# oksuman/FHE-Sorting

Hardware: AMD Instinct MI355X
Metric: encrypted sort seconds + ciphertext-mults/sec, N=1024 @ ringDim 2^16 (higher is better)
Workload: dtype u64; 1 GPU; DirectSort N=1024, ringDim 2^16, depth 39, scale 2^40, 161 rotation keys, CompositeSign(3, 5, 2), dnum 3, OpenFHE PS split; N=1024, ring_dim=65536, mult_depth=39, scale_bits=40, ps_split=openfhe, special_primes=10, lanes_per_gpu=2, max_stack=32, parallelism=batch-shard x1, collective=none

## Files before the change

### fhe-sorting_amd/csrc/capi/capi.cpp

```cpp
#include <hip/hip_runtime.h>
#include <rccl/rccl.h>
#include <sys/random.h>

#include <cerrno>
#include <cstdlib>
#include <cstring>
#include <map>
#include <memory>
#include <new>
#include <string>

#include "../../../include/fhe_gpu.h"
#include "../algo/bootstrap.hpp"
#include "../algo/fhesort.hpp"
#include "../device/kernels.hpp"
#include "../algo/kway.hpp"
#include "../engine/engine.hpp"
#include "../wire/wire.hpp"

using namespace fhe;

struct fhe_ctx {
    std::unique_ptr<Engine> eng;
    wire::CtxParams params;
// ... 158 lines not shown
    });
}
int fhe_key_is_seeded(fhe_ctx *ctx, uint64_t galois) {
    int r = -FHE_EINVAL;
    const int st = guard([&] {
        NEED(ctx);
        r = ctx->eng->key_seeded(galois);
        if (r < 0) {
            g_err = "fhe_key_is_seeded: no such key";
            r = -FHE_ENOKEY;
        }
    });
    return st == FHE_OK ? r : -st;
}
int fhe_public_poly(fhe_ctx *ctx, const uint8_t seed[32], uint64_t kid, int digit, uint64_t *out) {
    return guard([&] {
        NEED(ctx);
        NEED(seed);
        NEED(out);
        ctx->eng->public_poly(seed, kid, digit, out);
    });
}
uint64_t fhe_key_bytes(fhe_ctx *ctx) { return ctx ? ctx->eng->key_bytes() : 0; }

int fhe_encrypt(fhe_ctx *ctx, const double *v, int len, int slots, int level, fhe_ct **out) {
    return guard([&] { *out = wrap(ctx->eng->encrypt(std::vector<double>(v, v + len), slots, level)); });
}
int fhe_encrypt_ext(fhe_ctx *ctx, const double *v, int len, int slots, fhe_ct **out) {
    return guard([&] { *out = wrap(ctx->eng->encrypt_ext(std::vector<double>(v, v + len), slots)); });
}
int fhe_decrypt(fhe_ctx *ctx, const fhe_ct *ct, double *out) {
    return guard([&] {
        auto v = ctx->eng->decrypt(*ct->p);
        std::memcpy(out, v.data(), v.size() * 8);
    });
}
int fhe_ct_upload(fhe_ctx *ctx, const uint64_t *h, int limbs, int level, int slots, double scale, fhe_ct **out) {
    return guard([&] { *out = wrap(ctx->eng->upload(h, (size_t)limbs, level, slots, scale)); });
}
int fhe_ct_download(fhe_ctx *ctx, const fhe_ct *ct, uint64_t *h) {
    return guard([&] { ctx->eng->download(*ct->p, h); });
}
int fhe_ct_info(const fhe_ct *ct, int *level, int *slots, double *scale, int *limbs) {
    return guard([&] {
        NEED(ct);
        if (level) *level = ct->p->level;
// ... 1624 lines not shown
```

### fhe-sorting_amd/csrc/device/kernels.hpp

```cpp
#pragma once
#include <string>
#include <utility>
#include <vector>
#include <hip/hip_runtime.h>
#include <hip/hip_ext.h>
#include <cstddef>
#include <cstdint>

#include "modmath.hpp"

namespace fhe {
namespace dev {

struct NttTables {
    const ulonglong2 *fwd2;
    const ulonglong2 *inv2;
    const u64 *ninv, *ninv_s;
    const Mod *mods;
    int logN;
    const double *fwdd = nullptr, *invd = nullptr;
    const double2 *qd = nullptr;
    const uint8_t *fp_host = nullptr;
};
bool ntt_fp_prime(u64 q);
// ... 166 lines not shown

void encode_ifft(double2 *v, int64_t *coef, int B, int S, int n, const double2 *ksi, const uint32_t *rot,
                 const double *scale, unsigned *overflow, hipStream_t st);
void mask_slots(double2 *v, int B, int S, int N, const int *spec, hipStream_t st);
void select_slots(double2 *vc, double2 *vk, int S, int N, const int *targets, int count, int shift, hipStream_t st);
void tiebreak_slots(double2 *v, int B, int S, int N, const int *batches, double eps, hipStream_t st);

int set_mfma_sums(int mask);
void modup_convert(u64 *ext, const u64 *coef, int ell, int K, int alpha, int digits, int members,
                   size_t coef_stride, size_t ext_stride, const int *pmap_ext,
                   const u64 *tabs , const size_t *tab_off, const Mod *mods, int logN,
                   hipStream_t st,
                   const double *fptab = nullptr, const size_t *fp_off = nullptr, int fpmid = -1);
struct KsStrides {
    size_t acc = 0, ext = 0, d = 0;
    int zs0 = 0, zn0 = 1 << 30, zs1 = 0;
    __host__ __device__ int target_of(int z) const { return z < zn0 ? zs0 + z : zs1 + (z - zn0); }
};
struct KsFold {
    const u64 *d = nullptr;
    size_t seg = 0, member = 0;
    u64 w = 0, ws = 0;
};
void ks_inner(u64 *acc, const u64 *ext, const u64 *dntt, const u64 *key, int ell, int K, int nq, int nall,
              int alpha, int digits, const uint32_t *perm, const int *pmap_ext, const Mod *mods, int logN,
              hipStream_t st, int members, KsStrides str, KsFold fold = KsFold(), int tcount = -1);
void ntt_forward_mapped_cols(u64 *data, int count, int segs, size_t seg, const int *smap, const int *pmap,
                             const NttTables &T, hipStream_t st);
void ntt_row_ks(u64 *acc, const u64 *ext, const u64 *dntt, const u64 *key, int ell, int K, int nall, int alpha,
                int digits, const int *pmap_ext, int members, KsStrides str, KsFold fold, const NttTables &T,
                hipStream_t st, bool fp_only = false, int tfirst = 0);
void ntt_forward_mapped_rows(u64 *data, int count, int segs, size_t seg, const int *smap, const int *pmap,
                             const NttTables &T, hipStream_t st);
std::vector<std::pair<int, int>> ntt_class_runs(const int *pmap, int count, bool fp, const NttTables &T);
constexpr int KS_MAXKEYS = 16;
struct KsKeys {
    const u64 *key[KS_MAXKEYS];
    const uint32_t *perm[KS_MAXKEYS];
};
void ks_inner_multikey_sum(u64 *acc, const u64 *ext, const u64 *dntt, const KsKeys &keys, int count, bool accumulate,
                           int ell, int K, int nall, int alpha, int digits, const int *pmap_ext, const Mod *mods,
                           int logN, hipStream_t st, KsStrides str);
constexpr int LT_MAXB = 16;
struct LtArgs {
    const u64 *key[LT_MAXB];
    const uint32_t *perm[LT_MAXB];
    const u64 *pt[LT_MAXB];
    int nb;
};
void lt_inner(u64 *out, const u64 *ext, const u64 *c, const LtArgs &A, bool accumulate, int ell, int K, int nall,
              int alpha, int digits, const int *pmap_ext, const u64 *pmodq, const u64 *pmodq_s, const Mod *mods,
              int logN, hipStream_t st);
void ew_permute_sum(u64 *out, const u64 *in, const KsKeys &keys, int limbs, int count, bool accumulate, size_t in_stride,
                    const Mod *mods, int logN, hipStream_t st);
// ... 40 lines not shown
```

### fhe-sorting_amd/csrc/device/ntt.hip

```cpp
#include <hip/hip_ext.h>

#include <cstdlib>
#include <map>
#include <atomic>
#include <mutex>
#include <stdexcept>
#include <string>
#include <type_traits>
#include <utility>
#include <vector>

#include "kernels.hpp"

namespace fhe {
namespace dev {

namespace {

constexpr int NTB = 256;

template <int Lo, int Hi, typename F>
void dispatch_int(int v, F &&f) {
    if constexpr (Lo > Hi) {
        throw std::invalid_argument("unsupported digit count " + std::to_string(v));
// ... 879 lines not shown
#endif
#ifndef FHE_NTT_FP_ROW_WPE
#define FHE_NTT_FP_ROW_WPE 1
#endif
#ifndef FHE_NTT_FP_RESCALE_WPE
#define FHE_NTT_FP_RESCALE_WPE FHE_NTT_FP_ROW_WPE
#endif
template <int MODE, bool FULL, bool TWL, bool FP>
__global__ __launch_bounds__(NTB) __attribute__((amdgpu_waves_per_eu(FP ? (MODE == NTT_RESCALE ? FHE_NTT_FP_RESCALE_WPE : FHE_NTT_FP_ROW_WPE) : TWL ? FHE_NTT_ROW_WPE : 1, 8))) void k_ntt_fwd_row(
    u64 *data, size_t seg, const int *pmap, const int *smap, int logN, NttTables Tb, NttFuse F) {
    ntt_fwd_body<8, 4, false, MODE, true, FULL, TWL, FP>(data, seg, pmap, smap, logN, Tb, F, blockIdx.z);
}
template <bool FULL, bool TWL, bool FP>
__global__ __launch_bounds__(NTB) __attribute__((amdgpu_waves_per_eu(TWL ? FHE_NTT_ROW_WPE : 1, 8))) void k_ntt_inv_row(
    u64 *data, size_t seg, const int *pmap, const int *smap, int logN, NttTables Tb, NttFuse F) {
    ntt_inv_body<8, 4, false, true, FULL, TWL, FP>(data, seg, pmap, smap, logN, Tb, F);
}
#ifndef FHE_ROW_KS_WPE
#define FHE_ROW_KS_WPE 2
#endif
#ifndef FHE_ROW_KS_WPE1
#define FHE_ROW_KS_WPE1 4
#endif
template <int D, bool FP, bool FULL>
__global__ __launch_bounds__(NTB) __attribute__((amdgpu_waves_per_eu(D == 1 ? FHE_ROW_KS_WPE1 : FHE_ROW_KS_WPE, 8))) void k_ntt_row_ks(u64 *acc, const u64 *ext, const u64 *dntt, const u64 *key,
                                                    int ell, int W, int nall, int alpha, int members,
                                                    const int *pmap_ext, int logN, NttTables Tb, KsStrides st,
                                                    KsFold fold, NttFuse Fz, int lmb) {
    using TW = TwT<FP>;
    __shared__ TW twl[TWL_ROWS * 256];
    const size_t n = (size_t)1 << logN;
    const int t = Fz.limb_of(blockIdx.z);
    const int pt = __builtin_amdgcn_readfirstlane(pmap_ext[t]);
    const int tr = threadIdx.x >> 4, tl = threadIdx.x & 15;
    const int R = 16 >> lmb;
    const int mb = ((int)blockIdx.x << lmb) + (tr & ((1 << lmb) - 1));
    const bool valid = FULL || mb < members;
    const size_t row0 = (size_t)blockIdx.y * R, row = row0 + (tr >> lmb), rb = row * 256;
    const Mod md = Tb.mods[pt];
    const u64 q = md.q, q2 = 2 * q;
    Ar A{4 * q, (u64)0 - q, 0.0, 0.0};
    const TW *tw;
    if constexpr (FP) {
        tw = Tb.fwdd + (size_t)pt * n;
        const double2 qd = Tb.qd[pt];
        A.q = qd.x;
        A.qi = qd.y;
    } else {
        tw = Tb.fwd2 + (size_t)pt * n;
    }
    const int S0 = logN - 8;
    row_twiddles_multi<true>(twl, tw, row0, R, n, S0);
    __syncthreads();
    const TW *twr = twl + 256 * (tr >> lmb);
    const size_t m = valid ? (size_t)mb : 0;
    const int li = row_final_index<true>(tl, 0);
#define IDX(r) (li + (row_final_index<true>(0, r)))
    const bool folded = fold.d && t == ell - 1;
    const u64 *fd = fold.d + m * fold.member;
    auto digit_row = [&](int j, u64(&x)[16]) {
        const int lo = j * alpha, hi = min((j + 1) * alpha, ell);
        if (t >= lo && t < hi) {
            const u64 *src = dntt + m * st.d + (size_t)t * n + rb;
#pragma unroll
            for (int r = 0; r < 16; ++r) {
                const u64 v = valid ? src[IDX(r)] : 0;
                x[r] = FP ? ubits(fp_in(v, FP_TWO52)) : v;
            }
        } else {
            const u64 *src = ext + m * st.ext + ((size_t)j * W + t) * n + rb;
            const double fin = FP ? FP_TWO52 + FP_FWD_COL_OUT * A.q : 0.0;
#pragma unroll
            for (int r = 0; r < 16; ++r) {
                const u64 v = valid ? src[tl + 16 * r] : 0;
                x[r] = FP ? ubits(fp_in(v, fin)) : v;
            }
            row_pass_shfl<true, true, FP>(x, tl, row, twr, n, S0, A);
            if constexpr (!FP) {
#pragma unroll
                for (int r = 0; r < 16; ++r) x[r] = canon12(x[r], q, q2);
            }
        }
    };
    auto mac = [&](int j, const u64(&x)[16], u64(&a0)[16], u64(&a1)[16]) {
        const u64 *kb = key + (((size_t)j * 2 + 0) * nall + pt) * n + rb;
        const u64 *ka = key + (((size_t)j * 2 + 1) * nall + pt) * n + rb;
#pragma unroll
        for (int r = 0; r < 16; ++r) {
            const u64 b = kb[IDX(r)], c = ka[IDX(r)];
            if constexpr (FP) {
                const double xv = dbits(x[r]);
                a0[r] = ubits(dbits(a0[r]) + fp_mulmod(xv, fp_in(b, FP_TWO52), A.q, A.qi));
                a1[r] = ubits(dbits(a1[r]) + fp_mulmod(xv, fp_in(c, FP_TWO52), A.q, A.qi));
            } else {
                a0[r] = add_mod(a0[r], mul_barrett(x[r], b, md), q);
                a1[r] = add_mod(a1[r], mul_barrett(x[r], c, md), q);
            }
        }
    };
    auto fold_of = [&](int r, u64 &f0, u64 &f1) {
        f0 = f1 = 0;
        if (folded && valid) {
            f0 = mul_shoup(fd[rb + IDX(r)], fold.w, fold.ws, q);
            f1 = mul_shoup(fd[fold.seg + rb + IDX(r)], fold.w, fold.ws, q);
        }
    };
    u64 *o0 = acc + m * st.acc + (size_t)t * n + rb;
    u64 *o1 = acc + m * st.acc + ((size_t)W + t) * n + rb;
    auto fin = [&](u64 v) -> u64 {
        if constexpr (FP) {
            const double r0 = fp_reduce(dbits(v), A.q, A.qi);
            return fp_out(r0 < 0.0 ? r0 + A.q : r0, FP_TWO52);
        } else {
            return v;
        }
    };
    if constexpr (D == 1) {
        u64 x[16];
        digit_row(0, x);
        const u64 *kb = key + (size_t)pt * n + rb;
        const u64 *ka = key + ((size_t)nall + pt) * n + rb;
#pragma unroll
        for (int r = 0; r < 16; ++r) {
            u64 f0, f1, v0, v1;
            fold_of(r, f0, f1);
            const u64 b = kb[IDX(r)], c = ka[IDX(r)];
            if constexpr (FP) {
                const double xv = dbits(x[r]);
                v0 = ubits(fp_in(f0, FP_TWO52) + fp_mulmod(xv, fp_in(b, FP_TWO52), A.q, A.qi));
                v1 = ubits(fp_in(f1, FP_TWO52) + fp_mulmod(xv, fp_in(c, FP_TWO52), A.q, A.qi));
            } else {
                v0 = add_mod(f0, mul_barrett(x[r], b, md), q);
                v1 = add_mod(f1, mul_barrett(x[r], c, md), q);
            }
            if (valid) {
                o0[IDX(r)] = fin(v0);
                o1[IDX(r)] = fin(v1);
            }
        }
        return;
    }
    u64 a0[16], a1[16];
#pragma unroll
    for (int r = 0; r < 16; ++r) {
        u64 f0, f1;
        fold_of(r, f0, f1);
        a0[r] = FP ? ubits(fp_in(f0, FP_TWO52)) : f0;
        a1[r] = FP ? ubits(fp_in(f1, FP_TWO52)) : f1;
    }
#pragma unroll 1
    for (int j = 0; j < D; ++j) {
        u64 x[16];
        digit_row(j, x);
        mac(j, x, a0, a1);
    }
    if (!valid) return;
#pragma unroll
    for (int r = 0; r < 16; ++r) {
        o0[IDX(r)] = fin(a0[r]);
        o1[IDX(r)] = fin(a1[r]);
    }
#undef IDX
}

int &row_twl_enabled() {
    static int v = [] {
        const char *e = std::getenv("FHE_NTT_TWL");
        return e ? std::atoi(e) : 1;
    }();
    return v;
}

int &row_twl_rows() {
    static int v = [] {
        const char *e = std::getenv("FHE_NTT_TWL_ROWS");
        return e ? std::atoi(e) : 4;
    }();
    return v;
}
// ... 401 lines not shown
void ntt_forward_mapped_rows(u64 *data, int count, int segs, size_t seg, const int *smap, const int *pmap,
                             const NttTables &T, hipStream_t st) {
    if (count <= 0 || segs <= 0) return;
    const int k2 = T.logN - (T.logN + 1) / 2;
    const NttFuse F;
    dispatch<false, true, NTT_PLAIN>(k2, data, count, segs, seg, pmap, smap, T, F, st);
}

std::vector<std::pair<int, int>> ntt_class_runs(const int *pmap, int count, bool fp, const NttTables &T) {
    std::vector<int> pr;
    const bool known = launch_primes(pmap, count, pr);
    std::vector<std::pair<int, int>> runs;
    for (int z = 0; z < count; ++z) {
        const bool f = ntt_fp_enabled() && T.fp_host && known && T.fp_host[pr[z]] != 0;
        if (f != fp) continue;
        if (!runs.empty() && runs.back().first + runs.back().second == z) ++runs.back().second;
        else runs.emplace_back(z, 1);
    }
    return runs;
}

void ntt_row_ks(u64 *acc, const u64 *ext, const u64 *dntt, const u64 *key, int ell, int K, int nall, int alpha,
                int digits, const int *pmap_ext, int members, KsStrides str, KsFold fold, const NttTables &T,
                hipStream_t st, bool fp_only, int tfirst) {
    const int W = ell + K;
    if (T.logN != 16 && T.logN != 17) throw std::invalid_argument("ntt_row_ks: the row pass is 256 points (rings 2^16, 2^17)");
    if (digits < 1 || digits > 8) throw std::invalid_argument("ntt_row_ks: 1..8 digits");
    if (members < 1) return;
    std::vector<int> pr;
    const bool known = launch_primes(pmap_ext, W, pr);
    (void)pr;
    if (!known && ntt_fp_enabled() && T.fp_host) throw std::invalid_argument("ntt_row_ks: unregistered prime map");
    int lmb = 4;
    while (lmb > 2 && (1 << lmb) > members) --lmb;
    const bool full = members % (1 << lmb) == 0;
    const dim3 blk(NTB);
    for (int cls = fp_only ? 1 : 0; cls < 2; ++cls) {
        std::vector<std::pair<int, int>> runs;
        for (auto r : ntt_class_runs(pmap_ext, W, cls == 1, T)) {
            const int lo = std::max(r.first, tfirst), hi = r.first + r.second;
            if (lo < hi) runs.emplace_back(lo, hi - lo);
        }
        for (size_t r = 0; r < runs.size(); r += 2) {
            NttFuse Fz;
            Fz.zs0 = runs[r].first;
            Fz.zn0 = runs[r].second;
            Fz.zs1 = r + 1 < runs.size() ? runs[r + 1].first : 0;
            const int cnt = runs[r].second + (r + 1 < runs.size() ? runs[r + 1].second : 0);
            const dim3 grid((unsigned)((members + (1 << lmb) - 1) >> lmb), (unsigned)((1u << (T.logN - 8)) >> (4 - lmb)),
                            (unsigned)cnt);
            const double bytes = 8.0 * ((double)members * (digits + 2.0) + 2.0 * digits) * cnt * ((size_t)1 << T.logN);
            dispatch_int<1, 8>(digits, [&](auto c) {
                constexpr int DD = decltype(c)::value;
                auto go = [&](auto fpc, auto fullc) {
                    constexpr bool FPV = decltype(fpc)::value, FU = decltype(fullc)::value;
                    launch_clocked(inst_name<DD, FPV, FU>("k_ntt_row_ks"), bytes, k_ntt_row_ks<DD, FPV, FU>, grid, blk,
                                   st, acc, ext, dntt, key, ell, W, nall, alpha, members, pmap_ext, T.logN, T, str,
                                   fold, Fz, lmb);
                };
                if (cls && full) go(std::true_type{}, std::true_type{});
                else if (cls) go(std::true_type{}, std::false_type{});
                else if (full) go(std::false_type{}, std::true_type{});
                else go(std::false_type{}, std::false_type{});
            });
        }
    }
}

}
}
```

### fhe-sorting_amd/csrc/engine/engine.hip

```cpp
#include <hip/hip_runtime.h>

#include <algorithm>
#include <atomic>
#include <chrono>
#include <cmath>
#include <cstring>
#include <map>
#include <mutex>
#include <set>
#include <stdexcept>
#include <functional>
#include <thread>

#include "../device/kernels.hpp"
#include "engine.hpp"

#define HIP_OK(x)                                                                                     \
    do {                                                                                              \
        hipError_t _e = (x);                                                                          \
        if (_e != hipSuccess)                                                                         \
            throw std::runtime_error(std::string("HIP error ") + hipGetErrorString(_e) + " at " +    \
                                     __FILE__ + ":" + std::to_string(__LINE__));                      \
    } while (0)

// ... 130 lines not shown
    u64 *modup_tab = nullptr;
    u64 *phinv = nullptr, *phinv_s = nullptr, *phat = nullptr, *pinv = nullptr, *pinv_s = nullptr;
    u64 *qlinv = nullptr, *qlinv_s = nullptr;
    u64 *pmod = nullptr, *pmod_s = nullptr, *pqlinv = nullptr, *pqlinv_s = nullptr;
    double *pinvd = nullptr;
    double *mdfp_c = nullptr, *mdfp_q = nullptr;
    double *modup_fp = nullptr;
    int *modup_smap = nullptr, *modup_pmap = nullptr;
    struct FpState {
        std::vector<uint8_t> fp_host;
        std::vector<const int *> maps;
        void reg(const int *dev, const std::vector<int> &host) {
            dev::ntt_register_map(dev, host.data(), host.size());
            maps.push_back(dev);
        }
        ~FpState() {
            for (const int *m : maps) dev::ntt_unregister_map(m);
        }
    };
    std::shared_ptr<FpState> fps = std::make_shared<FpState>();

    struct KeySet {
        std::shared_ptr<DevMem> s_ntt, pk, relin;
        std::map<u64, std::shared_ptr<DevMem>> rotkeys;
        bool has_pub_seed = false;
        PublicSeed pub_seed{};
        std::map<u64, PublicSeed> seeded;
    };
    std::shared_ptr<DevMem> pub_err;
    std::shared_ptr<KeySet> ks = std::make_shared<KeySet>();
    std::map<u64, std::shared_ptr<DevMem>> perms;
    int key_digits = 0;

    struct ConstTab {
        std::shared_ptr<DevMem> mem;
        std::vector<int64_t> K;
        std::vector<uint8_t> sh;
        u64 used = 0;
    };
    std::map<std::string, ConstTab> ctabs;
    u64 ctab_tick = 0;
    std::pair<const int64_t *, const uint8_t *> const_table(const std::vector<int64_t> &K,
                                                           const std::vector<uint8_t> &sh) {
        std::string key(reinterpret_cast<const char *>(K.data()), K.size() * sizeof(int64_t));
        key.append(reinterpret_cast<const char *>(sh.data()), sh.size());
        key.append(std::to_string(K.size()));
// ... 129 lines not shown
            const char *e = std::getenv("FHE_KS_FUSE");
            return e ? std::atoi(e) : 1;
        }();
        static const int min_members = [] {
            const char *e = std::getenv("FHE_KS_FUSE_MIN");
            return e ? std::max(1, std::atoi(e)) : 4;
        }();
        return on && members >= min_members && (P.logN == 16 || P.logN == 17);
    }
    static bool ks_fuse_int() {
        static const bool on = [] {
            const char *e = std::getenv("FHE_KS_FUSE_INT");
            return e ? std::atoi(e) != 0 : true;
        }();
        return on;
    }
    static bool multail_own() {
        static const bool on = [] {
            const char *e = std::getenv("FHE_MULTAIL_OWN");
            return e ? std::atoi(e) != 0 : true;
        }();
        return on;
    }
    std::shared_ptr<DevMem> modup(const u64 *d, size_t ell, int members, size_t d_stride, bool cols_only = false) {
        Phase phase_("modup");
        const size_t nn = n(), K = (size_t)P.K, W = ell + K;
        const int digits = P.digits_at(ell);
        auto coef = alloc((size_t)members * ell * nn * 8);
        u64 *c = static_cast<u64 *>(coef->p);
        dev::ntt_inverse_from(c, d, d_stride, (int)ell, members, ell * nn, nullptr, T, st,  true);
        const size_t es = (size_t)digits * W * nn;
        auto extm = alloc((size_t)members * es * 8);
        u64 *e = static_cast<u64 *>(extm->p);
        dev::modup_convert(e, c, (int)ell, P.K, P.alpha, digits, members, ell * nn, es, ext(ell), modup_tab,
                           LT.modup_off[ell].data(), mods, P.logN, st, modup_fp, LT.modup_fp_off[ell].data(),
                           LT.modup_fp_mid);
        const size_t mo = LT.modup_map_off[ell];
        if (cols_only) {
            const int cnt = (int)LT.modup_map_cnt[ell];
            dev::ntt_forward_mapped_cols(e, cnt, members, es, modup_smap + mo, modup_pmap + mo, T, st);
            if (!ks_fuse_int())
            for (auto &r : dev::ntt_class_runs(modup_pmap + mo, cnt, false, T))
                dev::ntt_forward_mapped_rows(e, r.second, members, es, modup_smap + mo + r.first,
                                             modup_pmap + mo + r.first, T, st);
        } else
            dev::ntt_forward_mapped(e, (int)LT.modup_map_cnt[ell], members, es, modup_smap + mo, modup_pmap + mo, T, st);
// ... 54 lines not shown
        dev::ntt_forward_ksfinish(conv, (int)ell, segs, F, T, st);
    }
    void mul_tail(const u64 *e, const u64 *d01, const u64 *d2, size_t ell, int members, u64 *out, bool fused = false) {
        Phase phase_("mul_tail");
        const size_t nn = n(), K = (size_t)P.K, W = ell + K;
        const int digits = P.digits_at(ell);
        const int segs = 2 * members;
        auto accm = alloc((size_t)segs * W * nn * 8);
        u64 *acc = static_cast<u64 *>(accm->p);
        dev::KsStrides str;
        str.acc = 2 * W * nn;
        str.ext = (size_t)digits * W * nn;
        str.d = ell * nn;
        dev::KsFold fold;
        fold.d = d01 + (ell - 1) * nn;
        fold.seg = ell * nn;
        fold.member = 2 * ell * nn;
        fold.w = LT.pmod[ell - 1];
        fold.ws = LT.pmod_s[ell - 1];
        const bool own = fused && digits == 1 && ell >= 2 && ks_fuse_int() && multail_own();
        if (fused) {
            dev::ntt_row_ks(acc, e, d2, static_cast<u64 *>(ks->relin->p), (int)ell, P.K, (int)P.nall(), P.alpha, digits,
                            ext(ell), members, str, fold, T, st,  !ks_fuse_int(),
                             own ? (int)ell - 1 : 0);
            const auto runs = ks_fuse_int() ? std::vector<std::pair<int, int>>{}
                                            : dev::ntt_class_runs(ext(ell), (int)W, false, T);
            for (size_t r = 0; r < runs.size(); r += 2) {
                dev::KsStrides s2 = str;
                s2.zs0 = runs[r].first;
                s2.zn0 = runs[r].second;
                s2.zs1 = r + 1 < runs.size() ? runs[r + 1].first : 0;
                const int cnt = runs[r].second + (r + 1 < runs.size() ? runs[r + 1].second : 0);
                dev::ks_inner(acc, e, d2, static_cast<u64 *>(ks->relin->p), (int)ell, P.K, (int)P.nq(), (int)P.nall(),
                              P.alpha, digits, nullptr, ext(ell), mods, P.logN, st, members, s2, fold, cnt);
            }
        } else
            dev::ks_inner(acc, e, d2, static_cast<u64 *>(ks->relin->p), (int)ell, P.K, (int)P.nq(), (int)P.nall(),
                          P.alpha, digits, nullptr, ext(ell), mods, P.logN, st, members, str, fold);
        dev::ntt_inverse(acc + (ell - 1) * nn, (int)K + 1, segs, W * nn, ext(ell) + (ell - 1), T, st,  true);
        auto corrm = alloc((size_t)segs * (ell - 1) * nn * 8);
        u64 *corr = static_cast<u64 *>(corrm->p);
        dev::moddown_rescale_convert(corr, acc, (int)ell, P.K, (int)P.nq(), W * nn, (ell - 1) * nn, segs, phinv,
                                     phinv_s, phat, pinv, pinv_s, pmod, pinvd, T.ninv, T.ninv_s, mods, P.logN, st,
                                     pmod_s, mdfp_c, mdfp_q, LT.mdfp_mid);
        dev::NttFuse F;
        F.out = out;
        F.seg_out = (ell - 1) * nn;
// ... 246 lines not shown
        host::Prng g(I.ent, host::tags::pk_a, true);
        for (size_t l = 0; l < nq; ++l)
            for (size_t k = 0; k < n; ++k) a[l * n + k] = host::sample_uniform_mod(g, I.P.primes[l]);
    }
    auto e = sample_coeffs(I.ent, host::tags::pk_e, n, false);
    I.ks->pk = I.alloc(2 * nq * n * 8);
    u64 *pk = static_cast<u64 *>(I.ks->pk->p);
    HIP_OK(hipMemcpyAsync(pk + nq * n, a.data(), nq * n * 8, hipMemcpyHostToDevice, I.st));
    auto ec = I.alloc(n * 8);
    HIP_OK(hipMemcpyAsync(ec->p, e.data(), n * 8, hipMemcpyHostToDevice, I.st));
    auto tmp = I.alloc(nq * n * 8);
    u64 *t = static_cast<u64 *>(tmp->p);
    dev::ew_signed_to_rns(pk, static_cast<int64_t *>(ec->p), (int)nq, nullptr, I.mods, I.P.logN, I.st);
    dev::ntt_forward(pk, (int)nq, 1, 0, nullptr, I.T, I.st);
    dev::ew_mul_plain(t, pk + nq * n, S, (int)nq, 1, dev::Seg{0, 0, 0}, I.mods, I.P.logN, I.st);
    dev::ew_sub(pk, pk, t, (int)nq, 1, dev::Seg{0, 0, 0}, I.mods, I.P.logN, I.st);
    HIP_OK(hipStreamSynchronize(I.st));
    auto s2 = I.alloc(nq * n * 8);
    dev::ew_mul_plain(static_cast<u64 *>(s2->p), S, S, (int)nq, 1, dev::Seg{0, 0, 0}, I.mods, I.P.logN, I.st);
    I.ks->relin = I.alloc((size_t)I.key_digits * 2 * nall * n * 8);
    extern void gen_switch_key_impl(Engine::Impl &I, const u64 *sp, u64 kid, u64 *out);
    gen_switch_key_impl(I, static_cast<u64 *>(s2->p), 0, static_cast<u64 *>(I.ks->relin->p));
    HIP_OK(hipStreamSynchronize(I.st));
}

namespace {
void expand_public(Engine::Impl &I, const PublicSeed &seed, u64 kid, int digit, u64 *out) {
    if (!I.pub_err) {
        I.pub_err = I.alloc(sizeof(uint32_t));
        HIP_OK(hipMemsetAsync(I.pub_err->p, 0, sizeof(uint32_t), I.st));
    }
    uint32_t key[8];
    host::public_seed_key(seed.data(), key);
    dev::expand_uniform(out, key, (uint32_t)kid, digit, (int)I.P.nall(), I.mods, I.P.logN,
                        static_cast<uint32_t *>(I.pub_err->p), I.st);
}
void check_expansion(Engine::Impl &I, const PublicSeed &seed, u64 kid) {
    if (!I.pub_err) return;
    uint32_t err = 0;
    HIP_OK(hipMemcpyAsync(&err, I.pub_err->p, sizeof err, hipMemcpyDeviceToHost, I.st));
    HIP_OK(hipStreamSynchronize(I.st));
    if (!err) return;
    HIP_OK(hipMemsetAsync(I.pub_err->p, 0, sizeof(uint32_t), I.st));
    std::vector<u64> a(I.P.nall() * I.n());
    int bad = -1;
    for (int j = 0; j < I.key_digits && bad < 0; ++j)
// ... 92 lines not shown
}

void Engine::load_secret(const u64 *s) {
    auto &I = *impl;
    drain_before_key_load();
    const size_t bytes = I.P.nall() * I.n() * 8;
    I.ks->s_ntt = I.alloc(bytes);
    HIP_OK(hipMemcpy(I.ks->s_ntt->p, s, bytes, hipMemcpyHostToDevice));
}
void Engine::load_public(const u64 *pk) {
    auto &I = *impl;
    drain_before_key_load();
    const size_t bytes = 2 * I.P.nq() * I.n() * 8;
    I.ks->pk = I.alloc(bytes);
    HIP_OK(hipMemcpy(I.ks->pk->p, pk, bytes, hipMemcpyHostToDevice));
}
void Engine::load_relin(const u64 *key) {
    auto &I = *impl;
    drain_before_key_load();
    const size_t bytes = (size_t)I.key_digits * 2 * I.P.nall() * I.n() * 8;
    I.ks->relin = I.alloc(bytes);
    HIP_OK(hipMemcpy(I.ks->relin->p, key, bytes, hipMemcpyHostToDevice));
    I.ks->seeded.erase(0);
}
void Engine::load_rotation(long k, const u64 *key) {
    auto &I = *impl;
    drain_before_key_load();
    const size_t bytes = (size_t)I.key_digits * 2 * I.P.nall() * I.n() * 8;
    const u64 g = host::galois_for_rotation(I.P.logN, k);
    auto m = I.alloc(bytes);
    HIP_OK(hipMemcpy(m->p, key, bytes, hipMemcpyHostToDevice));
    I.ks->rotkeys[g] = m;
    I.ks->seeded.erase(g);
}
void Engine::load_galois(u64 g, const u64 *key) {
    auto &I = *impl;
    drain_before_key_load();
    const size_t bytes = (size_t)I.key_digits * 2 * I.P.nall() * I.n() * 8;
    auto m = I.alloc(bytes);
    HIP_OK(hipMemcpy(m->p, key, bytes, hipMemcpyHostToDevice));
    I.ks->rotkeys[g] = m;
    I.ks->seeded.erase(g);
}
namespace {
std::shared_ptr<DevMem> load_seeded_key(Engine::Impl &I, const PublicSeed &seed, u64 kid, const u64 *b) {
    drain_before_key_load();
    const size_t half = I.P.nall() * I.n();
    auto m = I.alloc((size_t)I.key_digits * 2 * half * 8);
    u64 *key = static_cast<u64 *>(m->p);
    HIP_OK(hipMemcpy2D(key, 2 * half * 8, b, half * 8, half * 8, (size_t)I.key_digits, hipMemcpyHostToDevice));
    for (int j = 0; j < I.key_digits; ++j) expand_public(I, seed, kid, j, key + ((size_t)j * 2 + 1) * half);
    check_expansion(I, seed, kid);
    return m;
}
}
void Engine::load_relin_seeded(const uint8_t seed[32], const u64 *b) {
    PublicSeed s;
    std::memcpy(s.data(), seed, 32);
    impl->ks->relin = load_seeded_key(*impl, s, 0, b);
    impl->ks->seeded[0] = s;
}
void Engine::load_galois_seeded(const uint8_t seed[32], u64 g, const u64 *b) {
    PublicSeed s;
    std::memcpy(s.data(), seed, 32);
    impl->ks->rotkeys[g] = load_seeded_key(*impl, s, g, b);
    impl->ks->seeded[g] = s;
}
void Engine::set_public_seed(const uint8_t seed[32]) {
    std::memcpy(impl->ks->pub_seed.data(), seed, 32);
    impl->ks->has_pub_seed = true;
}
bool Engine::get_public_seed(uint8_t seed[32]) const {
    if (!impl->ks->has_pub_seed) return false;
    std::memcpy(seed, impl->ks->pub_seed.data(), 32);
    return true;
}
int Engine::key_seeded(u64 kid, uint8_t *seed) const {
    const auto &K = *impl->ks;
    if (kid == 0 ? !K.relin : !K.rotkeys.count(kid)) return -1;
    auto it = K.seeded.find(kid);
    if (it == K.seeded.end()) return 0;
    if (seed) std::memcpy(seed, it->second.data(), 32);
    return 1;
// ... 32 lines not shown
std::vector<u64> Engine::galois_elements() const {
    std::vector<u64> gs;
    for (auto &kv : impl->ks->rotkeys) gs.push_back(kv.first);
    return gs;
}
void Engine::export_galois(u64 g, u64 *out) {
    auto it = impl->ks->rotkeys.find(g);
    if (it == impl->ks->rotkeys.end()) throw std::invalid_argument("export: no key for galois element " + std::to_string(g));
    export_key(*impl, it->second, switch_key_words(), out, "galois key");
}
namespace {
void export_key_b(Engine::Impl &I, const std::shared_ptr<DevMem> &m, u64 *out, const char *what) {
    if (!m) throw std::invalid_argument(std::string("export: no ") + what);
    const size_t half = I.P.nall() * I.n();
    HIP_OK(hipStreamSynchronize(I.st));
    HIP_OK(hipMemcpy2D(out, half * 8, m->p, 2 * half * 8, half * 8, (size_t)I.key_digits, hipMemcpyDeviceToHost));
}
}
void Engine::export_relin_b(u64 *out) { export_key_b(*impl, impl->ks->relin, out, "relinearisation key"); }
void Engine::export_galois_b(u64 g, u64 *out) {
    auto it = impl->ks->rotkeys.find(g);
    if (it == impl->ks->rotkeys.end()) throw std::invalid_argument("export: no key for galois element " + std::to_string(g));
    export_key_b(*impl, it->second, out, "galois key");
}
size_t Engine::key_bytes() const {
    size_t b = impl->ks->relin ? impl->ks->relin->bytes : 0;
    for (auto &kv : impl->ks->rotkeys) b += kv.second->bytes;
    return b;
}

PtPtr Engine::encode(const std::vector<double> &v, int slots, int level) {
    return encode_scaled(v, slots, level, impl->P.delta[level]);
}
PtPtr Engine::encode_scaled(const std::vector<double> &v, int slots, int level, double scale) {
    auto &I = *impl;
    const u64 t0 = now_ns();
    const size_t n = I.n(), ell = I.P.limbs_at(level);
    auto coef = host::encode_coeffs(v, n, slots, scale);
    auto cm = I.alloc(n * 8);
    HIP_OK(hipMemcpyAsync(cm->p, coef.data(), n * 8, hipMemcpyHostToDevice, I.st));
    auto pt = std::make_shared<Plaintext>();
    pt->mem = I.alloc(ell * n * 8);
    pt->data = static_cast<u64 *>(pt->mem->p);
    pt->level = level;
    pt->slots = slots;
    pt->scale = scale;
// ... 2162 lines not shown
```

### fhe-sorting_amd/csrc/engine/engine.hpp

```cpp
#pragma once
#include <array>
#include <complex>
#include <cstddef>
#include <cstdint>
#include <memory>
#include <stdexcept>
#include <string>
#include <vector>

#include "../host/hostmath.hpp"

namespace fhe {

using u64 = uint64_t;
using i64 = int64_t;
using PublicSeed = std::array<uint8_t, 32>;

struct DevMem;

struct Ciphertext {
    std::shared_ptr<DevMem> mem;
    u64 *data = nullptr;
    int level = 0;
    int slots = 0;
// ... 50 lines not shown
    const host::Params &params() const;
    size_t n() const;
    double delta(int level) const;

    void keygen();
    void gen_rotation_keys(const std::vector<int> &rot);
    void load_secret(const u64 *s_ntt);
    void load_public(const u64 *pk);
    void load_relin(const u64 *key);
    void load_rotation(long k, const u64 *key);
    bool has_rotation_key(long k) const;
    void gen_galois_keys(const std::vector<u64> &gs);
    void load_galois(u64 g, const u64 *key);
    bool has_galois_key(u64 g) const;
    size_t key_bytes() const;
    int key_digits() const;
    size_t switch_key_words() const;
    bool has_secret() const;
    bool has_public() const;
    bool has_relin() const;
    void export_secret(u64 *out);
    void export_public(u64 *out);
    void export_relin(u64 *out);
    std::vector<u64> galois_elements() const;
    void export_galois(u64 g, u64 *out);
    void set_public_seed(const uint8_t seed[32]);
    bool get_public_seed(uint8_t seed[32]) const;
    int key_seeded(u64 kid, uint8_t *seed = nullptr) const;
    void public_poly(const uint8_t seed[32], u64 kid, int digit, u64 *out);
    void export_relin_b(u64 *out);
    void export_galois_b(u64 g, u64 *out);
    void load_relin_seeded(const uint8_t seed[32], const u64 *b);
    void load_galois_seeded(const uint8_t seed[32], u64 g, const u64 *b);

    PtPtr encode(const std::vector<double> &v, int slots, int level);
    PtPtr encode_scaled(const std::vector<double> &v, int slots, int level, double scale);
    PtPtr encode_complex(const std::vector<std::complex<double>> &v, int slots, int level, double scale);
    PtPtr encode_complex_ext(const std::vector<std::complex<double>> &v, int slots, int level, double scale);
    struct MaskSpec {
        int kind, k, r, level;
    };
    std::vector<PtPtr> encode_masks(const std::vector<MaskSpec> &specs, int num_slots, int N);
    std::vector<PtPtr> encode_device(const std::vector<std::vector<double>> &vs, int slots, const std::vector<int> &levels);
    std::array<PtPtr, 2> encode_select(const std::vector<int> &targets, int member, int num_slots, int N, int level_c,
                                       int level_k);
    static std::vector<double> tiebreak_offsets(int N, int num_slots, int batch, double eps);
// ... 139 lines not shown
```

### fhe-sorting_amd/fhesort.py

```python
import ctypes as C
import os

import numpy as np

HERE = os.path.dirname(os.path.abspath(__file__))
LIB_PATH = os.environ.get('FHE_LIB') or os.path.join(HERE, 'lib', 'libfhesort.so')
COEFF_DIR = os.path.join(HERE, 'data')
HEADER = os.path.join(os.path.dirname(HERE), 'include', 'fhe_gpu.h')
PS_SPLIT_ENGINE, PS_SPLIT_OPENFHE = 0, 1
RUN_ROWS, RUN_LE, RUN_LT, RUN_BETWEEN = range(4)
WIN_ROWS, WIN_LE, WIN_LT, WIN_BETWEEN, WIN_GROUP = range(5)

FHE_OK, FHE_EINVAL, FHE_ENOKEY, FHE_EDEPTH, FHE_EHIP, FHE_ENOMEM, FHE_EINTERNAL, FHE_ENOCOMM, FHE_EIO = range(9)
NAF, BNAF, BINARY = 0, 1, 2
SORT_COLUMN_MEMBERS_DEFAULT = 256
TENSOR_COLS_PER_THREAD = 4
PLAIN_SUM_GROUPS_PER_THREAD = 4


class FheError(RuntimeError):
    def __init__(self, code, msg):
        super().__init__(f'fhe error {code}: {msg}')
        self.code = code

# ... 27 lines not shown
                return 1
        self.fn = ALLREDUCE_FN(call) if f else None

    def ptr(self):
        return C.cast(self.fn, C.c_void_p) if self.fn else None

    def reraise(self, err):
        if self.exc is not None:
            raise self.exc from err
        raise err

_SIGS = {
    'fhe_last_error': (C.c_char_p, []),
    'fhe_ctx_create': (C.c_int, [C.POINTER(Params), C.c_int, PP]),
    'fhe_ctx_destroy': (C.c_int, [vp]),
    'fhe_ctx_info': (C.c_int, [vp, ip, ip, ip, u64p, dp]),
    'fhe_set_coeff_dir': (C.c_int, [C.c_char_p]),
    'fhe_keygen': (C.c_int, [vp]),
    'fhe_gen_rotation_keys': (C.c_int, [vp, ip, C.c_int]),
    'fhe_ctx_load_secret': (C.c_int, [vp, u64p]),
    'fhe_ctx_load_public': (C.c_int, [vp, u64p]),
    'fhe_ctx_load_keys': (C.c_int, [vp, u64p, ip, C.POINTER(u64p), C.c_int]),
    'fhe_key_bytes': (C.c_uint64, [vp]),
    'fhe_encrypt': (C.c_int, [vp, dp, C.c_int, C.c_int, C.c_int, PP]),
    'fhe_encrypt_ext': (C.c_int, [vp, dp, C.c_int, C.c_int, PP]),
    'fhe_decrypt': (C.c_int, [vp, vp, dp]),
    'fhe_ct_upload': (C.c_int, [vp, u64p, C.c_int, C.c_int, C.c_int, C.c_double, PP]),
    'fhe_ct_download': (C.c_int, [vp, vp, u64p]),
    'fhe_ct_info': (C.c_int, [vp, ip, ip, dp, ip]),
    'fhe_ct_set_slots': (C.c_int, [vp, C.c_int]),
    'fhe_ct_free': (C.c_int, [vp]),
    'fhe_pt_encode': (C.c_int, [vp, dp, C.c_int, C.c_int, C.c_int, PP]),
    'fhe_pt_upload': (C.c_int, [vp, u64p, C.c_int, C.c_int, C.c_int, C.c_double, PP]),
    'fhe_pt_free': (C.c_int, [vp]),
    'fhe_add': (C.c_int, [vp, vp, vp, PP]),
    'fhe_sub': (C.c_int, [vp, vp, vp, PP]),
    'fhe_negate': (C.c_int, [vp, vp, PP]),
    'fhe_add_const': (C.c_int, [vp, vp, C.c_double, PP]),
    'fhe_mul_const': (C.c_int, [vp, vp, C.c_double, PP]),
    'fhe_mul_const_to': (C.c_int, [vp, vp, C.c_double, C.c_int, PP]),
    'fhe_mul_int': (C.c_int, [vp, vp, C.c_int64, PP]),
    'fhe_level_adjust': (C.c_int, [vp, vp, C.c_int, PP]),
    'fhe_rescale': (C.c_int, [vp, vp, PP]),
    'fhe_mul_plain': (C.c_int, [vp, vp, vp, PP]),
    'fhe_add_plain': (C.c_int, [vp, vp, vp, PP]),
    'fhe_mul_relin': (C.c_int, [vp, vp, vp, PP]),
# ... 451 lines not shown
        keys, idx = [], []
        for k in rots:
            g, key = orc.rot_key(k)
            if g:
                keys.append(np.ascontiguousarray(key))
                idx.append(k)
        arr = (u64p * max(1, len(keys)))(*[_u64(k) for k in keys])
        ia = np.asarray(idx, dtype=np.int32)
        _chk(lib().fhe_ctx_load_keys(self.h, _u64(rl), _int(ia), arr, len(keys)))

    def load_galois_keys_from(self, orc, gs):
        for g in gs:
            key = orc.galois_key(g)
            if key is not None:
                _chk(lib().fhe_ctx_load_galois_key(self.h, int(g), _u64(np.ascontiguousarray(key))))

    def gen_galois_keys(self, gs):
        g = np.asarray(gs, dtype=np.uint64)
        _chk(lib().fhe_gen_galois_keys(self.h, _u64(g), len(g)))

    def key_bytes(self):
        return lib().fhe_key_bytes(self.h)

    def set_public_seed(self, seed=None):
        if seed is not None:
            seed = bytes(seed)
            if len(seed) != 32:
                raise ValueError('a public seed is 32 bytes')
        _chk(lib().fhe_set_public_seed(self.h, seed))

    def get_public_seed(self):
        buf = C.create_string_buffer(32)
        _chk(lib().fhe_get_public_seed(self.h, buf))
        return buf.raw

    def key_is_seeded(self, galois=0):
        r = lib().fhe_key_is_seeded(self.h, int(galois))
        if r < 0:
            _chk(-r)
        return r

    def public_poly(self, seed, kid, digit):
        seed = bytes(seed)
        if len(seed) != 32:
            raise ValueError('a public seed is 32 bytes')
        out = np.empty((self.nq + self.K, self.n), dtype=np.uint64)
# ... 688 lines not shown
```

### include/fhe_gpu.h

```cpp
#ifndef FHE_GPU_H
#define FHE_GPU_H

#include <stdint.h>

#ifdef __cplusplus
extern "C" {
#endif

enum {
    FHE_OK = 0,
    FHE_EINVAL = 1,
    FHE_ENOKEY = 2,
    FHE_EDEPTH = 3,
    FHE_EHIP = 4,
    FHE_ENOMEM = 5,
    FHE_EINTERNAL = 6,
    FHE_ENOCOMM = 7,
    FHE_EIO = 8
};

typedef struct fhe_ctx fhe_ctx;
typedef struct fhe_ct fhe_ct;
typedef struct fhe_pt fhe_pt;
typedef struct fhe_boot fhe_boot;
// ... 2 lines not shown
    int log_n;
    int mult_depth;
    int scale_bits;
    int first_bits;
    int dnum;
    uint64_t seed;
} fhe_params;

const char *fhe_last_error(void);
int fhe_prng_block(const uint32_t key[8], uint32_t counter, const uint32_t nonce[3], uint32_t out[16]);

int fhe_ctx_create(const fhe_params *p, int device, fhe_ctx **out);
int fhe_ctx_destroy(fhe_ctx *ctx);
int fhe_ctx_info(fhe_ctx *ctx, int *nq, int *K, int *alpha, uint64_t *primes, double *deltas);
int fhe_set_coeff_dir(const char *dir);

int fhe_keygen(fhe_ctx *ctx);
int fhe_gen_rotation_keys(fhe_ctx *ctx, const int32_t *idx, int n);
int fhe_ctx_load_secret(fhe_ctx *ctx, const uint64_t *s_ntt);
int fhe_ctx_load_public(fhe_ctx *ctx, const uint64_t *pk);
int fhe_ctx_load_keys(fhe_ctx *ctx, const uint64_t *relin, const int32_t *rot_idx,
                      const uint64_t *const *rot_keys, int nrot);
uint64_t fhe_key_bytes(fhe_ctx *ctx);
int fhe_set_public_seed(fhe_ctx *ctx, const uint8_t seed[32]);
int fhe_get_public_seed(fhe_ctx *ctx, uint8_t seed[32]);
int fhe_key_is_seeded(fhe_ctx *ctx, uint64_t galois );

int fhe_encrypt(fhe_ctx *ctx, const double *v, int len, int slots, int level, fhe_ct **out);
int fhe_encrypt_ext(fhe_ctx *ctx, const double *v, int len, int slots, fhe_ct **out);
int fhe_decrypt(fhe_ctx *ctx, const fhe_ct *ct, double *out);
int fhe_ct_upload(fhe_ctx *ctx, const uint64_t *host, int limbs, int level, int slots, double scale,
                  fhe_ct **out);
int fhe_ct_download(fhe_ctx *ctx, const fhe_ct *ct, uint64_t *host);
int fhe_ct_info(const fhe_ct *ct, int *level, int *slots, double *scale, int *limbs);
int fhe_ct_set_slots(fhe_ct *ct, int slots);
int fhe_ct_free(fhe_ct *ct);
int fhe_mul_plain_sum(fhe_ctx *ctx, const fhe_ct *const *cts, const fhe_pt *const *pts, int m, fhe_ct **out);
int fhe_mul_plain_sum_batches(fhe_ctx *ctx, const fhe_ct *const *cts, const fhe_pt *const *pts, int m, int nb,
                              fhe_ct **out);
int fhe_plain_sum_tile(void);
double fhe_plain_sum_batches_limb_units(int m, int nb, int tile);
int fhe_ct_stack(fhe_ctx *ctx, const fhe_ct *const *xs, int m, fhe_ct **out);
int fhe_ct_member(fhe_ctx *ctx, const fhe_ct *a, int m, fhe_ct **out);
int fhe_ct_sum_members(fhe_ctx *ctx, const fhe_ct *a, fhe_ct **out);
int fhe_pt_encode(fhe_ctx *ctx, const double *v, int len, int slots, int level, fhe_pt **out);
int fhe_pt_upload(fhe_ctx *ctx, const uint64_t *host, int limbs, int level, int slots, double scale,
// ... 241 lines not shown
```

Before: 11310 ciphertext-mults/s.

## Precompute Shoup companions for relinearisation key in fused single-digit row keyswitch

Builds, at key load or generation time, Shoup precomputed companions (floor(k*2^64/q)) for the relinearisation key rows used by the single-digit fused NTT-row keyswitch. The integer path then multiplies the lazily reduced digit values against the key using Shoup multiplication, skipping the per-row canonical reduction and a full modular reduction per product. It also raises the waves-per-EU hint for the integer single-digit instantiation. In exchange it reads an extra companion array per key element, adding memory traffic and extra device memory, and it adds export APIs for the companions.

```diff
diff --git a/fhe-sorting_amd/csrc/capi/capi.cpp b/fhe-sorting_amd/csrc/capi/capi.cpp
--- a/fhe-sorting_amd/csrc/capi/capi.cpp
+++ b/fhe-sorting_amd/csrc/capi/capi.cpp
@@ -204,6 +204,15 @@
     });
 }
 uint64_t fhe_key_bytes(fhe_ctx *ctx) { return ctx ? ctx->eng->key_bytes() : 0; }
+uint64_t fhe_relin_shoup_bytes(fhe_ctx *ctx) { return ctx ? ctx->eng->relin_shoup_bytes() : 0; }
+uint64_t fhe_relin_shoup_words(fhe_ctx *ctx) { return ctx ? ctx->eng->relin_shoup_words() : 0; }
+int fhe_export_relin_shoup(fhe_ctx *ctx, uint64_t *out) {
+    return guard([&] {
+        NEED(ctx);
+        NEED(out);
+        ctx->eng->export_relin_shoup(out);
+    });
+}
 
 int fhe_encrypt(fhe_ctx *ctx, const double *v, int len, int slots, int level, fhe_ct **out) {
     return guard([&] { *out = wrap(ctx->eng->encrypt(std::vector<double>(v, v + len), slots, level)); });
diff --git a/fhe-sorting_amd/csrc/device/kernels.hpp b/fhe-sorting_amd/csrc/device/kernels.hpp
--- a/fhe-sorting_amd/csrc/device/kernels.hpp
+++ b/fhe-sorting_amd/csrc/device/kernels.hpp
@@ -212,6 +212,11 @@
     size_t seg = 0, member = 0;
     u64 w = 0, ws = 0;
 };
+struct KsShoup {
+    const u64 *w = nullptr;
+    const int *cmap = nullptr;
+    int rows = 0;
+};
 void ks_inner(u64 *acc, const u64 *ext, const u64 *dntt, const u64 *key, int ell, int K, int nq, int nall,
               int alpha, int digits, const uint32_t *perm, const int *pmap_ext, const Mod *mods, int logN,
               hipStream_t st, int members, KsStrides str, KsFold fold = KsFold(), int tcount = -1);
@@ -219,7 +224,9 @@
                              const NttTables &T, hipStream_t st);
 void ntt_row_ks(u64 *acc, const u64 *ext, const u64 *dntt, const u64 *key, int ell, int K, int nall, int alpha,
                 int digits, const int *pmap_ext, int members, KsStrides str, KsFold fold, const NttTables &T,
-                hipStream_t st, bool fp_only = false, int tfirst = 0);
+                hipStream_t st, bool fp_only = false, int tfirst = 0, KsShoup shoup = KsShoup());
+void relin_shoup_build(u64 *sh, const u64 *key, const int *cmap, int rows, int digits, int nall, const Mod *mods,
+                       int logN, hipStream_t st);
 void ntt_forward_mapped_rows(u64 *data, int count, int segs, size_t seg, const int *smap, const int *pmap,
                              const NttTables &T, hipStream_t st);
 std::vector<std::pair<int, int>> ntt_class_runs(const int *pmap, int count, bool fp, const NttTables &T);
diff --git a/fhe-sorting_amd/csrc/device/ntt.hip b/fhe-sorting_amd/csrc/device/ntt.hip
--- a/fhe-sorting_amd/csrc/device/ntt.hip
+++ b/fhe-sorting_amd/csrc/device/ntt.hip
@@ -925,11 +925,14 @@
 #ifndef FHE_ROW_KS_WPE1
 #define FHE_ROW_KS_WPE1 4
 #endif
+#ifndef FHE_ROW_KS_WPE1_INT
+#define FHE_ROW_KS_WPE1_INT 5
+#endif
 template <int D, bool FP, bool FULL>
-__global__ __launch_bounds__(NTB) __attribute__((amdgpu_waves_per_eu(D == 1 ? FHE_ROW_KS_WPE1 : FHE_ROW_KS_WPE, 8))) void k_ntt_row_ks(u64 *acc, const u64 *ext, const u64 *dntt, const u64 *key,
+__global__ __launch_bounds__(NTB) __attribute__((amdgpu_waves_per_eu(D == 1 ? (FP ? FHE_ROW_KS_WPE1 : FHE_ROW_KS_WPE1_INT) : FHE_ROW_KS_WPE, 8))) void k_ntt_row_ks(u64 *acc, const u64 *ext, const u64 *dntt, const u64 *key,
                                                     int ell, int W, int nall, int alpha, int members,
                                                     const int *pmap_ext, int logN, NttTables Tb, KsStrides st,
-                                                    KsFold fold, NttFuse Fz, int lmb) {
+                                                    KsFold fold, NttFuse Fz, int lmb, KsShoup sh) {
     using TW = TwT<FP>;
     __shared__ TW twl[TWL_ROWS * 256];
     const size_t n = (size_t)1 << logN;
@@ -961,7 +964,7 @@
 #define IDX(r) (li + (row_final_index<true>(0, r)))
     const bool folded = fold.d && t == ell - 1;
     const u64 *fd = fold.d + m * fold.member;
-    auto digit_row = [&](int j, u64(&x)[16]) {
+    auto digit_row = [&](int j, u64(&x)[16], auto lazy) {
         const int lo = j * alpha, hi = min((j + 1) * alpha, ell);
         if (t >= lo && t < hi) {
             const u64 *src = dntt + m * st.d + (size_t)t * n + rb;
@@ -979,7 +982,7 @@
                 x[r] = FP ? ubits(fp_in(v, fin)) : v;
             }
             row_pass_shfl<true, true, FP>(x, tl, row, twr, n, S0, A);
-            if constexpr (!FP) {
+            if constexpr (!FP && !decltype(lazy)::value) {
 #pragma unroll
                 for (int r = 0; r < 16; ++r) x[r] = canon12(x[r], q, q2);
             }
@@ -1008,8 +1011,7 @@
             f1 = mul_shoup(fd[fold.seg + rb + IDX(r)], fold.w, fold.ws, q);
         }
     };
-    u64 *o0 = acc + m * st.acc + (size_t)t * n + rb;
-    u64 *o1 = acc + m * st.acc + ((size_t)W + t) * n + rb;
+    auto out0 = [&] { return acc + m * st.acc + (size_t)t * n + rb; };
     auto fin = [&](u64 v) -> u64 {
         if constexpr (FP) {
             const double r0 = fp_reduce(dbits(v), A.q, A.qi);
@@ -1018,9 +1020,37 @@
             return v;
         }
     };
+    if constexpr (!FP && D == 1) {
+        const int cr = sh.w ? __builtin_amdgcn_readfirstlane(sh.cmap[pt]) : -1;
+        if (cr >= 0) {
+            const size_t half = (size_t)sh.rows * n;
+            u64 x[16];
+            digit_row(0, x, std::true_type{});
+            u64 *o0 = out0(), *o1 = o0 + (size_t)W * n;
+            const u64 *kb = key + (size_t)pt * n, *ka = kb + (size_t)nall * n;
+            const u64 *cb = sh.w + (size_t)cr * n, *ca = cb + half;
+            const unsigned lo = (unsigned)rb + (unsigned)li;
+#define KIX(r) ((size_t)lo + (row_final_index<true>(0, r)))
+#pragma unroll
+            for (int r = 0; r < 16; ++r) {
+                u64 f0, f1;
+                fold_of(r, f0, f1);
+                const u64 v0 = f0 + shoup_fold4(x[r], kb[KIX(r)], cb[KIX(r)], A.nq);
+                const u64 v1 = f1 + shoup_fold4(x[r], ka[KIX(r)], ca[KIX(r)], A.nq);
+                if (valid) {
+                    o0[IDX(r)] = canon8(v0, q, q2);
+                    o1[IDX(r)] = canon8(v1, q, q2);
+                }
+                if (r % 4 == 3) __builtin_amdgcn_sched_barrier(0);
+            }
+#undef KIX
+            return;
+        }
+    }
     if constexpr (D == 1) {
         u64 x[16];
-        digit_row(0, x);
+        digit_row(0, x, std::false_type{});
+        u64 *o0 = out0(), *o1 = o0 + (size_t)W * n;
         const u64 *kb = key + (size_t)pt * n + rb;
         const u64 *ka = key + ((size_t)nall + pt) * n + rb;
 #pragma unroll
@@ -1054,10 +1084,11 @@
 #pragma unroll 1
     for (int j = 0; j < D; ++j) {
         u64 x[16];
-        digit_row(j, x);
+        digit_row(j, x, std::false_type{});
         mac(j, x, a0, a1);
     }
     if (!valid) return;
+    u64 *o0 = out0(), *o1 = o0 + (size_t)W * n;
 #pragma unroll
     for (int r = 0; r < 16; ++r) {
         o0[IDX(r)] = fin(a0[r]);
@@ -1505,7 +1536,7 @@
 
 void ntt_row_ks(u64 *acc, const u64 *ext, const u64 *dntt, const u64 *key, int ell, int K, int nall, int alpha,
                 int digits, const int *pmap_ext, int members, KsStrides str, KsFold fold, const NttTables &T,
-                hipStream_t st, bool fp_only, int tfirst) {
+                hipStream_t st, bool fp_only, int tfirst, KsShoup shoup) {
     const int W = ell + K;
     if (T.logN != 16 && T.logN != 17) throw std::invalid_argument("ntt_row_ks: the row pass is 256 points (rings 2^16, 2^17)");
     if (digits < 1 || digits > 8) throw std::invalid_argument("ntt_row_ks: 1..8 digits");
@@ -1539,7 +1570,7 @@
                     constexpr bool FPV = decltype(fpc)::value, FU = decltype(fullc)::value;
                     launch_clocked(inst_name<DD, FPV, FU>("k_ntt_row_ks"), bytes, k_ntt_row_ks<DD, FPV, FU>, grid, blk,
                                    st, acc, ext, dntt, key, ell, W, nall, alpha, members, pmap_ext, T.logN, T, str,
-                                   fold, Fz, lmb);
+                                   fold, Fz, lmb, shoup);
                 };
                 if (cls && full) go(std::true_type{}, std::true_type{});
                 else if (cls) go(std::true_type{}, std::false_type{});
@@ -1550,5 +1581,34 @@
     }
 }
 
-}
-}
+__global__ __launch_bounds__(256) void k_relin_shoup(u64 *sh, const u64 *key, const int *cmap, int rows, int nall,
+                                                     const Mod *mods, int logN) {
+    const size_t n = (size_t)1 << logN;
+    const int p = blockIdx.y;
+    const int cr = __builtin_amdgcn_readfirstlane(cmap[p]);
+    if (cr < 0 || cr >= rows) return;
+    const size_t k = (size_t)blockIdx.x * 256 + threadIdx.x;
+    if (k >= n) return;
+    const u64 q = mods[p].q;
+    u64 r = key[((size_t)blockIdx.z * nall + p) * n + k], w = 0;
+#pragma unroll 8
+    for (int i = 0; i < 64; ++i) {
+        r += r;
+        const bool ge = r >= q;
+        r = ge ? r - q : r;
+        w = (w << 1) | (u64)ge;
+    }
+    sh[((size_t)blockIdx.z * rows + cr) * n + k] = w;
+}
+
+void relin_shoup_build(u64 *sh, const u64 *key, const int *cmap, int rows, int digits, int nall, const Mod *mods,
+                       int logN, hipStream_t st) {
+    if (rows <= 0 || digits <= 0) return;
+    const size_t n = (size_t)1 << logN;
+    const dim3 grid((unsigned)((n + 255) / 256), (unsigned)nall, (unsigned)(2 * digits));
+    launch_clocked("k_relin_shoup", 16.0 * 2 * digits * rows * n, k_relin_shoup, grid, dim3(256), st, sh, key, cmap, rows,
+                   nall, mods, logN);
+}
+
+}
+}
diff --git a/fhe-sorting_amd/csrc/engine/engine.hip b/fhe-sorting_amd/csrc/engine/engine.hip
--- a/fhe-sorting_amd/csrc/engine/engine.hip
+++ b/fhe-sorting_amd/csrc/engine/engine.hip
@@ -176,6 +176,7 @@
 
     struct KeySet {
         std::shared_ptr<DevMem> s_ntt, pk, relin;
+        std::shared_ptr<DevMem> relin_shoup, relin_cmap;
         std::map<u64, std::shared_ptr<DevMem>> rotkeys;
         bool has_pub_seed = false;
         PublicSeed pub_seed{};
@@ -351,6 +352,38 @@
         }();
         return on;
     }
+    static bool relin_shoup_on() {
+        static const bool on = [] {
+            const char *e = std::getenv("FHE_RELIN_SHOUP");
+            return e ? std::atoi(e) != 0 : true;
+        }();
+        return on;
+    }
+    void build_relin_shoup() {
+        ks->relin_shoup.reset();
+        if (!relin_shoup_on() || !ks->relin) return;
+        const size_t nq = P.nq(), nall = P.nall(), rows = 1 + (size_t)P.K;
+        std::vector<int> cmap(nall, -1);
+        cmap[0] = 0;
+        for (size_t k = 0; k < (size_t)P.K; ++k) cmap[nq + k] = 1 + (int)k;
+        ks->relin_cmap = alloc(nall * sizeof(int));
+        HIP_OK(hipMemcpyAsync(ks->relin_cmap->p, cmap.data(), nall * sizeof(int), hipMemcpyHostToDevice, st));
+        auto sh = alloc((size_t)2 * rows * n() * 8);
+        dev::relin_shoup_build(static_cast<u64 *>(sh->p), static_cast<const u64 *>(ks->relin->p),
+                               static_cast<const int *>(ks->relin_cmap->p), (int)rows,  1, (int)nall, mods,
+                               P.logN, st);
+        HIP_OK(hipStreamSynchronize(st));
+        ks->relin_shoup = sh;
+    }
+    dev::KsShoup relin_shoup() const {
+        dev::KsShoup s;
+        if (ks->relin_shoup) {
+            s.w = static_cast<const u64 *>(ks->relin_shoup->p);
+            s.cmap = static_cast<const int *>(ks->relin_cmap->p);
+            s.rows = 1 + P.K;
+        }
+        return s;
+    }
     std::shared_ptr<DevMem> modup(const u64 *d, size_t ell, int members, size_t d_stride, bool cols_only = false) {
         Phase phase_("modup");
         const size_t nn = n(), K = (size_t)P.K, W = ell + K;
@@ -451,7 +484,7 @@
         if (fused) {
             dev::ntt_row_ks(acc, e, d2, static_cast<u64 *>(ks->relin->p), (int)ell, P.K, (int)P.nall(), P.alpha, digits,
                             ext(ell), members, str, fold, T, st,  !ks_fuse_int(),
-                             own ? (int)ell - 1 : 0);
+                             own ? (int)ell - 1 : 0, relin_shoup());
             const auto runs = ks_fuse_int() ? std::vector<std::pair<int, int>>{}
                                             : dev::ntt_class_runs(ext(ell), (int)W, false, T);
             for (size_t r = 0; r < runs.size(); r += 2) {
@@ -744,6 +777,7 @@
     extern void gen_switch_key_impl(Engine::Impl &I, const u64 *sp, u64 kid, u64 *out);
     gen_switch_key_impl(I, static_cast<u64 *>(s2->p), 0, static_cast<u64 *>(I.ks->relin->p));
     HIP_OK(hipStreamSynchronize(I.st));
+    I.build_relin_shoup();
 }
 
 namespace {
@@ -882,6 +916,7 @@
     I.ks->relin = I.alloc(bytes);
     HIP_OK(hipMemcpy(I.ks->relin->p, key, bytes, hipMemcpyHostToDevice));
     I.ks->seeded.erase(0);
+    I.build_relin_shoup();
 }
 void Engine::load_rotation(long k, const u64 *key) {
     auto &I = *impl;
@@ -919,6 +954,7 @@
     std::memcpy(s.data(), seed, 32);
     impl->ks->relin = load_seeded_key(*impl, s, 0, b);
     impl->ks->seeded[0] = s;
+    impl->build_relin_shoup();
 }
 void Engine::load_galois_seeded(const uint8_t seed[32], u64 g, const u64 *b) {
     PublicSeed s;
@@ -997,6 +1033,13 @@
     auto it = impl->ks->rotkeys.find(g);
     if (it == impl->ks->rotkeys.end()) throw std::invalid_argument("export: no key for galois element " + std::to_string(g));
     export_key_b(*impl, it->second, out, "galois key");
+}
+size_t Engine::relin_shoup_words() const {
+    return impl->ks->relin_shoup ? 2 * (1 + (size_t)impl->P.K) * impl->P.n : 0;
+}
+size_t Engine::relin_shoup_bytes() const { return impl->ks->relin_shoup ? impl->ks->relin_shoup->bytes : 0; }
+void Engine::export_relin_shoup(u64 *out) {
+    export_key(*impl, impl->ks->relin_shoup, relin_shoup_words(), out, "relinearisation key companions");
 }
 size_t Engine::key_bytes() const {
     size_t b = impl->ks->relin ? impl->ks->relin->bytes : 0;
diff --git a/fhe-sorting_amd/csrc/engine/engine.hpp b/fhe-sorting_amd/csrc/engine/engine.hpp
--- a/fhe-sorting_amd/csrc/engine/engine.hpp
+++ b/fhe-sorting_amd/csrc/engine/engine.hpp
@@ -96,6 +96,9 @@
     void export_secret(u64 *out);
     void export_public(u64 *out);
     void export_relin(u64 *out);
+    size_t relin_shoup_words() const;
+    size_t relin_shoup_bytes() const;
+    void export_relin_shoup(u64 *out);
     std::vector<u64> galois_elements() const;
     void export_galois(u64 g, u64 *out);
     void set_public_seed(const uint8_t seed[32]);
diff --git a/fhe-sorting_amd/fhesort.py b/fhe-sorting_amd/fhesort.py
--- a/fhe-sorting_amd/fhesort.py
+++ b/fhe-sorting_amd/fhesort.py
@@ -73,6 +73,9 @@
     'fhe_ctx_load_public': (C.c_int, [vp, u64p]),
     'fhe_ctx_load_keys': (C.c_int, [vp, u64p, ip, C.POINTER(u64p), C.c_int]),
     'fhe_key_bytes': (C.c_uint64, [vp]),
+    'fhe_relin_shoup_bytes': (C.c_uint64, [vp]),
+    'fhe_relin_shoup_words': (C.c_uint64, [vp]),
+    'fhe_export_relin_shoup': (C.c_int, [vp, u64p]),
     'fhe_encrypt': (C.c_int, [vp, dp, C.c_int, C.c_int, C.c_int, PP]),
     'fhe_encrypt_ext': (C.c_int, [vp, dp, C.c_int, C.c_int, PP]),
     'fhe_decrypt': (C.c_int, [vp, vp, dp]),
@@ -570,6 +573,14 @@
     def key_bytes(self):
         return lib().fhe_key_bytes(self.h)
 
+    def relin_shoup_bytes(self):
+        return lib().fhe_relin_shoup_bytes(self.h)
+
+    def export_relin_shoup(self):
+        out = np.empty(lib().fhe_relin_shoup_words(self.h), dtype=np.uint64)
+        _chk(lib().fhe_export_relin_shoup(self.h, _u64(out)))
+        return out.reshape(2, 1 + self.K, self.n)
+
     def set_public_seed(self, seed=None):
         if seed is not None:
             seed = bytes(seed)
diff --git a/include/fhe_gpu.h b/include/fhe_gpu.h
--- a/include/fhe_gpu.h
+++ b/include/fhe_gpu.h
@@ -48,6 +48,9 @@
 int fhe_ctx_load_keys(fhe_ctx *ctx, const uint64_t *relin, const int32_t *rot_idx,
                       const uint64_t *const *rot_keys, int nrot);
 uint64_t fhe_key_bytes(fhe_ctx *ctx);
+uint64_t fhe_relin_shoup_bytes(fhe_ctx *ctx);
+uint64_t fhe_relin_shoup_words(fhe_ctx *ctx);
+int fhe_export_relin_shoup(fhe_ctx *ctx, uint64_t *out);
 int fhe_set_public_seed(fhe_ctx *ctx, const uint8_t seed[32]);
 int fhe_get_public_seed(fhe_ctx *ctx, uint8_t seed[32]);
 int fhe_key_is_seeded(fhe_ctx *ctx, uint64_t galois );
```

Measured after the change: 11350 ciphertext-mults/s (median of 6 runs). Within noise of the previous version (+0.4%).
